# ilovin/lstm_ctc_ocr

Hardware: NVIDIA H100
Metric: text-line images/sec (fwd+CTC loss) (higher is better)
Workload: dtype bf16

## Files before the change

### lstm_ctc_ocr_b200/csrc/backward.cu

```cuda
#include <cmath>
#include <cstring>

#include "backward_kernels.cuh"
#include "conv1_wgrad_tc.cuh"
#include "conv_swap.cuh"
#include "gemm_launch.h"
#include "kernels.cuh"
#include "lstm_bwd.cuh"
#include "model_internal.h"

extern "C" int crnn_model_set_training(crnn_model* m, int flag) {
  if (!m) return crnn_fail(CRNN_INVALID_VALUE, "set_training: null model");
  if (flag && m->cfg.compute_dtype >= 2) return crnn_fail(CRNN_UNSUPPORTED, "set_training: the f32-class paths (compute_dtype 2, 3) are forward + CTC only");
  if (flag && !m->wblock_bwd) {
    const size_t nB[9] = {512 * 4608, 256 * 4608, 256 * 2304, 128 * 2304, 64 * 1152, 1024 * 1024, 512 * 64, 512 * 2048, 512 * 1024};
    size_t tot = 1024;
    for (size_t v : nB) tot += align_up(v * 2);
    CUDA_TRY(cudaMalloc(&m->wblock_bwd, tot));
    uint8_t* p = reinterpret_cast<uint8_t*>(m->wblock_bwd);
    __nv_bfloat16** dst[9] = {&m->Bd_c42, &m->Bd_c41, &m->Bd_c32, &m->Bd_c31, &m->Bd_c2, &m->Bd_c5, &m->Bld, &m->Bxb, &m->Bhb};
    for (int i = 0; i < 9; ++i) { *dst[i] = reinterpret_cast<__nv_bfloat16*>(p); p += align_up(nB[i] * 2); }
    m->grad_sumsq = reinterpret_cast<double*>(p);
    CRNN_TRY(make_tmap_2d(&m->tD_c42, m->Bd_c42, 512, 4608, 4608, 256));
    CRNN_TRY(make_tmap_2d(&m->tD_c41, m->Bd_c41, 256, 4608, 4608, 256));
    CRNN_TRY(make_tmap_2d(&m->tD_c32, m->Bd_c32, 256, 2304, 2304, 256));
    CRNN_TRY(make_tmap_2d(&m->tD_c31, m->Bd_c31, 128, 2304, 2304, 128));
    CRNN_TRY(make_tmap_2d(&m->tD_c2, m->Bd_c2, 64, 1152, 1152, 64));
    CRNN_TRY(make_tmap_2d(&m->tDs_c2, m->Bd_c2, 64, 1152, 1152, 128));
    CRNN_TRY(make_tmap_2d(&m->tD_c5, m->Bd_c5, 1024, 1024, 1024, 256));
    CRNN_TRY(make_tmap_2d(&m->tD_l, m->Bld, 512, 64, 64, 256));
    CRNN_TRY(make_tmap_2d(&m->tD_x, m->Bxb, 512, 2048, 2048, 256));
    CRNN_TRY(make_tmap_2d(&m->tD_h, m->Bhb, 512, 1024, 1024, 32));
    CRNN_TRY(make_tmap_2d(&m->tD_h256, m->Bhb, 512, 1024, 1024, 256));
    m->dirty_bwd = true;
  }
  m->training = flag != 0;
  return CRNN_OK;
}

static int prepare_weights_bwd(crnn_model* m, cudaStream_t st) {
  CRNN_TRY(launch_dgrad_weight(m->P("conv4_2/weights"), m->Bd_c42, 512, 512, st));
  CRNN_TRY(launch_dgrad_weight(m->P("conv4_1/weights"), m->Bd_c41, 256, 512, st));
  CRNN_TRY(launch_dgrad_weight(m->P("conv3_2/weights"), m->Bd_c32, 256, 256, st));
  CRNN_TRY(launch_dgrad_weight(m->P("conv3_1/weights"), m->Bd_c31, 128, 256, st));
  CRNN_TRY(launch_dgrad_weight(m->P("conv2/weights"), m->Bd_c2, 64, 128, st));
  CRNN_TRY(launch_conv5_dgrad_weight(m->P("conv5/weights"), m->Bd_c5, st));
  CRNN_TRY(launch_cast_bf16(m->P("logits/weights"), m->Bld, 512 * 64, st));
  CRNN_TRY(launch_lstm_bwd_weight(m->P("logits/bidirectional_rnn/fw/lstm_cell/weights"), m->P("logits/bidirectional_rnn/bw/lstm_cell/weights"),
                                  m->Bxb, m->Bhb, 32, st));
  m->dirty_bwd = false;
  return CRNN_OK;
}

static gemm_tn::Params tn_plain(int M, int Ncols, long long rows, float* out, long long ldo) {
  gemm_tn::Params p;
  memset(&p, 0, sizeof(p));
  p.num_taps = 1;
  p.num_m_tiles = (M + 127) / 128;
// ... 349 lines not shown
```

### lstm_ctc_ocr_b200/csrc/forward_x3.cu

```cuda
#include <cstring>
#include <string>

#include "gemm_launch.h"
#include "kernels.cuh"
#include "model_internal.h"

namespace x3 {

__device__ __forceinline__ void split2(float v, __nv_bfloat16& hi, __nv_bfloat16& lo) {
  hi = __float2bfloat16_rn(v);
  lo = __float2bfloat16_rn(v - __bfloat162float(hi));
}

__device__ __forceinline__ uint2 pack4(const __nv_bfloat16* h) {
  uint2 r;
  r.x = (uint32_t)__bfloat16_as_ushort(h[0]) | ((uint32_t)__bfloat16_as_ushort(h[1]) << 16);
  r.y = (uint32_t)__bfloat16_as_ushort(h[2]) | ((uint32_t)__bfloat16_as_ushort(h[3]) << 16);
  return r;
}

__global__ void __launch_bounds__(256) split_weight_kernel(const float* __restrict__ src, int K, int Cout, int ld, int inner,
                                                           __nv_bfloat16* __restrict__ dst) {
  const size_t i = (size_t)blockIdx.x * blockDim.x + threadIdx.x;
  if (i >= (size_t)K * Cout) return;
// ... 236 lines not shown
    CRNN_TRY(make_tmap_2d_f32(&pl.tA_l, pl.slo, Rt, 512, 512, 128));
    CRNN_TRY(make_tmap_2d_f32(&pl.tA_h, pl.hS, (uint64_t)2 * pl.Npad, 256, 256, 128));
    return CRNN_OK;
  }
  CRNN_TRY(make_tmap_nhwc(&pl.tA_c2, pl.s1, N, pl.H1, 16, 128, pl.mg2 ? 8 : 2));
  CRNN_TRY(make_tmap_nhwc(&pl.tA_c31, pl.s2, N, pl.H2, 8, 256, pl.mg3 ? 16 : 4));
  CRNN_TRY(make_tmap_nhwc(&pl.tA_c32, pl.s3, N, pl.H2, 8, 512, pl.mg3 ? 16 : 4));
  CRNN_TRY(make_tmap_nhwc(&pl.tA_c41, pl.s3p, N, pl.H2, 4, 512, pl.mg4 ? 32 : 8));
  CRNN_TRY(make_tmap_nhwc(&pl.tA_c42, pl.s4a, N, pl.H2, 4, 1024, pl.mg4 ? 32 : 8));
  const uint64_t R = (uint64_t)N * pl.H2;
  CRNN_TRY(make_tmap_2d(&pl.tA_c5, pl.s4b, R, 2048, 2048, 128));
  CRNN_TRY(make_tmap_2d(&pl.tA_x, pl.s5, R, 1024, 1024, 128));
  CRNN_TRY(make_tmap_2d(&pl.tA_l, pl.slo, R, 1024, 1024, 128));
  CRNN_TRY(make_tmap_2d(&pl.tA_h, pl.hS, (uint64_t)2 * pl.Npad, 512, 512, 128));
  return CRNN_OK;
}

static int prepare(crnn_model* m, State* s, cudaStream_t st) {
  const int kK[9] = {576, 1152, 2304, 2304, 4608, 2048, 512, 256, 512};
  const int kCo[9] = {128, 256, 256, 512, 512, 512, 2048, 2048, 64};
  if (!s->wblock) {
    const size_t eb = s->tf32 ? 4 : 6;
    size_t tot = 0;
    for (int i = 0; i < 9; ++i) tot += align_up((size_t)kK[i] * kCo[i] * eb);
    CUDA_TRY(cudaMalloc(&s->wblock, tot));
    uint8_t* p = reinterpret_cast<uint8_t*>(s->wblock);
    uint8_t** dst[9] = {&s->Bc2, &s->Bc31, &s->Bc32, &s->Bc41, &s->Bc42, &s->Bc5, &s->Bx, &s->Bh, &s->Bl};
    for (int i = 0; i < 9; ++i) { *dst[i] = p; p += align_up((size_t)kK[i] * kCo[i] * eb); }
  }
  if (s->tf32) {
    if (!s->maps_ready) {
      CUtensorMap* tm[9] = {&s->tB_c2, &s->tB_c31, &s->tB_c32, &s->tB_c41, &s->tB_c42, &s->tB_c5, &s->tB_x, &s->tB_h, &s->tB_l};
      uint8_t* base[9] = {s->Bc2, s->Bc31, s->Bc32, s->Bc41, s->Bc42, s->Bc5, s->Bx, s->Bh, s->Bl};
      const int box[9] = {128, 256, 256, 256, 256, 256, 256, 256, 64};
      for (int i = 0; i < 9; ++i) CRNN_TRY(make_tmap_2d_f32(tm[i], base[i], kCo[i], kK[i], kK[i], box[i]));
      s->maps_ready = true;
    }
    auto tw = [&](const float* src, int K, int Cout, int ld, uint8_t* dst) -> int {
      const size_t n = (size_t)K * Cout;
      tf32_weight_kernel<<<(unsigned)((n + 255) / 256), 256, 0, st>>>(src, K, Cout, ld, reinterpret_cast<float*>(dst));
      CUDA_TRY(cudaGetLastError());
      return CRNN_OK;
    };
    CRNN_TRY(tw(m->P("conv2/weights"), 576, 128, 128, s->Bc2));
    CRNN_TRY(tw(m->P("conv3_1/weights"), 1152, 256, 256, s->Bc31));
    CRNN_TRY(tw(m->P("conv3_2/weights"), 2304, 256, 256, s->Bc32));
    CRNN_TRY(tw(m->P("conv4_1/weights"), 2304, 512, 512, s->Bc41));
    CRNN_TRY(tw(m->P("conv4_2/weights"), 4608, 512, 512, s->Bc42));
    CRNN_TRY(tw(m->P("conv5/weights"), 2048, 512, 512, s->Bc5));
    const char* dn[2] = {"logits/bidirectional_rnn/fw/lstm_cell/weights", "logits/bidirectional_rnn/bw/lstm_cell/weights"};
    for (int d = 0; d < 2; ++d) {
      const float* w = m->P(dn[d]);
      CRNN_TRY(tw(w, 512, 1024, 1024, s->Bx + (size_t)d * 1024 * 512 * 4));
      CRNN_TRY(tw(w + 512 * 1024, 256, 1024, 1024, s->Bh + (size_t)d * 1024 * 256 * 4));
    }
    CRNN_TRY(tw(m->P("logits/weights"), 512, 64, 64, s->Bl));
    s->dirty = false;
    return CRNN_OK;
  }
  if (!s->maps_ready) {
    s->maps_ready = true;
    CRNN_TRY(make_tmap_2d(&s->tB_c2, s->Bc2, 128, 1728, 1728, 128));
    CRNN_TRY(make_tmap_2d(&s->tB_c31, s->Bc31, 256, 3456, 3456, 256));
    CRNN_TRY(make_tmap_2d(&s->tB_c32, s->Bc32, 256, 6912, 6912, 256));
    CRNN_TRY(make_tmap_2d(&s->tB_c41, s->Bc41, 512, 6912, 6912, 256));
    CRNN_TRY(make_tmap_2d(&s->tB_c42, s->Bc42, 512, 13824, 13824, 256));
    CRNN_TRY(make_tmap_2d(&s->tB_c5, s->Bc5, 512, 6144, 6144, 256));
    CRNN_TRY(make_tmap_2d(&s->tB_x, s->Bx, 2048, 1536, 1536, 256));
    CRNN_TRY(make_tmap_2d(&s->tB_h, s->Bh, 2048, 768, 768, 256));
    CRNN_TRY(make_tmap_2d(&s->tB_l, s->Bl, 64, 1536, 1536, 64));
  }
  auto sw = [&](const float* src, int K, int Cout, int ld, int inner, uint8_t* dst) -> int {
    const size_t n = (size_t)K * Cout;
    split_weight_kernel<<<(unsigned)((n + 255) / 256), 256, 0, st>>>(src, K, Cout, ld, inner, reinterpret_cast<__nv_bfloat16*>(dst));
    CUDA_TRY(cudaGetLastError());
    return CRNN_OK;
  };
  CRNN_TRY(sw(m->P("conv2/weights"), 576, 128, 128, 64, s->Bc2));
  CRNN_TRY(sw(m->P("conv3_1/weights"), 1152, 256, 256, 128, s->Bc31));
  CRNN_TRY(sw(m->P("conv3_2/weights"), 2304, 256, 256, 256, s->Bc32));
  CRNN_TRY(sw(m->P("conv4_1/weights"), 2304, 512, 512, 256, s->Bc41));
  CRNN_TRY(sw(m->P("conv4_2/weights"), 4608, 512, 512, 512, s->Bc42));
  CRNN_TRY(sw(m->P("conv5/weights"), 2048, 512, 512, 1024, s->Bc5));
  const char* dirs[2] = {"logits/bidirectional_rnn/fw/lstm_cell/weights", "logits/bidirectional_rnn/bw/lstm_cell/weights"};
  for (int d = 0; d < 2; ++d) {
    const float* w = m->P(dirs[d]);
    CRNN_TRY(sw(w, 512, 1024, 1024, 512, s->Bx + (size_t)d * 1024 * 1536 * 2));
    CRNN_TRY(sw(w + 512 * 1024, 256, 1024, 1024, 256, s->Bh + (size_t)d * 1024 * 768 * 2));
  }
  CRNN_TRY(sw(m->P("logits/weights"), 512, 64, 64, 512, s->Bl));
  s->dirty = false;
  return CRNN_OK;
}

template <int POOL>
static int act_split(bool tf, const float* in, void* out, const float* bias, const float* scale, const float* shift, int relu, int Nimg,
                     int H, int Wd, int C, int G, cudaStream_t st) {
  const int Ho = (POOL == 1) ? H / 2 : H, Wo = (POOL != 0) ? Wd / 2 : Wd;
  const size_t total = (size_t)Nimg * Ho * Wo * (C / 4);
// ... 187 lines not shown
```

### lstm_ctc_ocr_b200/csrc/gemm.cuh

```cuda
#pragma once
#include <cuda.h>

#include "common.cuh"
#include "wgmma.cuh"

namespace gemm {

constexpr int BLOCK_M = 128;
constexpr int BLOCK_K = 64;
constexpr int UMMA_K = 16;
constexpr int A_STAGE_BYTES = BLOCK_M * 128;
constexpr int NUM_THREADS = 384;
constexpr int MAX_SMEM = 232448;

enum AMode { A_PLAIN = 0, A_CONV3 = 1 };
enum Epi {
  EPI_F32 = 0,
  EPI_BIAS_BF16 = 1,
  EPI_RELU = 2,
  EPI_RELU_POOL22 = 3,
  EPI_RELU_POOL12 = 4,
  EPI_STATS = 5,
  EPI_LSTM = 6,
  EPI_LOGITS = 7,
// ... 55 lines not shown
  for (int i = 0; i < 4; ++i) {
    float send = (lane & 4) ? r8[i] : r8[i + 4];
    float keep = (lane & 4) ? r8[i + 4] : r8[i];
    r4[i] = keep + __shfl_xor_sync(0xffffffffu, send, 4);
  }
#pragma unroll
  for (int i = 0; i < 2; ++i) {
    float send = (lane & 2) ? r4[i] : r4[i + 2];
    float keep = (lane & 2) ? r4[i + 2] : r4[i];
    r2[i] = keep + __shfl_xor_sync(0xffffffffu, send, 2);
  }
  float send = (lane & 1) ? r2[0] : r2[1];
  float keep = (lane & 1) ? r2[1] : r2[0];
  return keep + __shfl_xor_sync(0xffffffffu, send, 1);
}

constexpr int slice_cols(int block_n, int epi) {
  return (block_n < 256 || epi == EPI_LSTM || epi == EPI_CONV_STORE_BNRED) ? block_n
       : (epi == EPI_RELU || epi == EPI_STATS || epi == EPI_BIAS_BF16 || epi == EPI_XPROJ || epi == EPI_CONV_STORE) ? 128 : 64;
}

template <int BLOCK_N, int STAGES, int SLICE_N>
struct Smem {
  static constexpr int B_STAGE_BYTES = BLOCK_N * 128;
  static constexpr int ACC_BYTES = BLOCK_M * SLICE_N * 4;
  static constexpr int FIT = (MAX_SMEM - ACC_BYTES - 256 - 1024) / (A_STAGE_BYTES + B_STAGE_BYTES);
  static constexpr int S = STAGES < FIT ? STAGES : FIT;
  static constexpr int ACC_OFFSET = S * (A_STAGE_BYTES + B_STAGE_BYTES);
  static constexpr int BAR_OFFSET = ACC_OFFSET + ACC_BYTES;
  static constexpr int BYTES = BAR_OFFSET + 256 + 1024;
};
static_assert(Smem<256, 4, 64>::S == 4, "a 64-column staging slice leaves room for a 4-stage ring at BLOCK_N = 256");

constexpr bool frag_epi(int block_n, int epi) {
  return block_n == 256 && (epi == EPI_RELU || epi == EPI_RELU_POOL12 || epi == EPI_STATS || epi == EPI_BIAS_BF16 ||
                            epi == EPI_XPROJ || epi == EPI_CONV_STORE);
}

__device__ __forceinline__ uint32_t* stg_word(uint8_t* buf, int box_bytes, int row, int c) {
  return reinterpret_cast<uint32_t*>(buf + (c >> 6) * box_bytes + row * 128 + ((((c >> 3) & 7) ^ (row & 7)) << 4) + ((c & 7) << 1));
}

template <int W>
__device__ __forceinline__ float4 rowsum_tree(const uint8_t* box, int rg, int cw, int i) {
  if constexpr (W == 32) {
    const int r = rg * 32 + i;
    const uint32_t v = *reinterpret_cast<const uint32_t*>(box + r * 128 + (((cw >> 2) ^ (r & 7)) << 4) + ((cw & 3) << 2));
    const float x = ptx::bf16_lo(v), y = ptx::bf16_hi(v);
    return make_float4(x, y, __fmul_rn(x, x), __fmul_rn(y, y));
  } else {
    const float4 a = rowsum_tree<W * 2>(box, rg, cw, i), b = rowsum_tree<W * 2>(box, rg, cw, i + W);
    return make_float4(a.x + b.x, a.y + b.y, a.z + b.z, a.w + b.w);
  }
}

template <bool LINES>
__device__ __forceinline__ bool conv_row_valid(const Params& p, int m_blk, int r) {
  const int g = m_blk * 4 + (r >> 5);
  const int n_img = g / p.sb_per_img;
  const int h = (g - n_img * p.sb_per_img) * p.bh + (r & 31) / p.Wd;
  if (LINES) return n_img < p.Nimg && h < (__ldg(p.line_w + n_img) >> 2);
  return n_img < p.Nimg && h < p.H;
}

template <int EPI, bool LINES = false>
__device__ __forceinline__ void frag_epilogue(const Params& p, const float (&d)[128], uint8_t* stg, const CUtensorMap* tmO,
// ... 456 lines not shown
        const uint32_t* xfw = reinterpret_cast<const uint32_t*>(xf);
        const uint32_t* xow = reinterpret_cast<const uint32_t*>(xo);
        float* cpf = reinterpret_cast<float*>(cp);
        float hv[16];
#pragma unroll
        for (int i = 0; i < 16; ++i) {
          const float zi = __uint_as_float(gi[i]) + ((i & 1) ? ptx::bf16_hi(xiw[i >> 1]) : ptx::bf16_lo(xiw[i >> 1]));
          const float zj = __uint_as_float(gj[i]) + ((i & 1) ? ptx::bf16_hi(xjw[i >> 1]) : ptx::bf16_lo(xjw[i >> 1]));
          const float zf = __uint_as_float(gf[i]) + ((i & 1) ? ptx::bf16_hi(xfw[i >> 1]) : ptx::bf16_lo(xfw[i >> 1]));
          const float zo = __uint_as_float(go[i]) + ((i & 1) ? ptx::bf16_hi(xow[i >> 1]) : ptx::bf16_lo(xow[i >> 1]));
          const float c = ptx::fast_sigmoid(zf) * cpf[i] + ptx::fast_sigmoid(zi) * ptx::fast_tanh(zj);
          cpf[i] = c;
          hv[i] = ptx::fast_sigmoid(zo) * ptx::fast_tanh(c);
        }
#pragma unroll
        for (int i = 0; i < 4; ++i) *(reinterpret_cast<float4*>(cst + u0) + i) = cp[i];
#pragma unroll
        for (int i = 0; i < 8; ++i) hp[i] = ptx::pack_bf16x2(hv[2 * i], hv[2 * i + 1]);
      } else {
#pragma unroll
        for (int i = 0; i < 8; ++i) hp[i] = 0u;
      }
      if (okn) {
        *reinterpret_cast<uint4*>(hn + u0) = make_uint4(hp[0], hp[1], hp[2], hp[3]);
        *reinterpret_cast<uint4*>(hn + u0 + 8) = make_uint4(hp[4], hp[5], hp[6], hp[7]);
        *reinterpret_cast<uint4*>(lo + u0) = make_uint4(hp[0], hp[1], hp[2], hp[3]);
        *reinterpret_cast<uint4*>(lo + u0 + 8) = make_uint4(hp[4], hp[5], hp[6], hp[7]);
      }
    }
  }

}

template <int BLOCK_N, int AMODE, int EPI, int STAGES, int KIND = 0, bool LINES = false>
__global__ void __launch_bounds__(NUM_THREADS, 1)
gemm_kernel(const __grid_constant__ CUtensorMap tmA, const __grid_constant__ CUtensorMap tmB, const __grid_constant__ CUtensorMap tmO,
            const Params p) {
  static_assert(BLOCK_N == 64 || BLOCK_N == 128 || BLOCK_N == 256, "BLOCK_N");
  constexpr bool FRAG = frag_epi(BLOCK_N, EPI);
  static_assert(!LINES || (FRAG && AMODE == A_CONV3 && KIND == 0), "line masks exist in the register-side conv epilogues only");
  constexpr int SLICE_N = slice_cols(BLOCK_N, EPI);
  using SM = Smem<BLOCK_N, STAGES, SLICE_N>;
  constexpr int S = SM::S;
  constexpr int B_STAGE_BYTES = BLOCK_N * 128;
  constexpr int KELEMS = KIND ? 32 : BLOCK_K;

  extern __shared__ uint8_t smem_raw[];
  uint8_t* smem = reinterpret_cast<uint8_t*>((reinterpret_cast<uintptr_t>(smem_raw) + 1023) & ~uintptr_t(1023));
  uint8_t* smem_a = smem;
  uint8_t* smem_b = smem + S * A_STAGE_BYTES;
  float* acc_tile = reinterpret_cast<float*>(smem + SM::ACC_OFFSET);
  uint64_t* full_bar = reinterpret_cast<uint64_t*>(smem + SM::BAR_OFFSET);
  uint64_t* empty_bar = full_bar + S;

  const int warp_idx = threadIdx.x >> 5;
  const int lane = threadIdx.x & 31;
  const int num_tiles = p.num_m_tiles * p.num_n_tiles;

  if (warp_idx == 0 && lane == 0) {
    ptx::prefetch_tmap(&tmA);
    ptx::prefetch_tmap(&tmB);
    if (FRAG) ptx::prefetch_tmap(&tmO);
    for (int s = 0; s < S; ++s) {
      ptx::mbar_init(&full_bar[s], 1);
      ptx::mbar_init(&empty_bar[s], 2);
    }
    ptx::fence_barrier_init();
  }
  __syncthreads();

  if (warp_idx < 4) {
    ptx::setmaxnreg_dec<24>();
    const int nA = (AMODE == A_CONV3 && !p.merged) ? 4 : 1;
    if (warp_idx == 0 && lane <= nA) {
      int stage = 0;
      uint32_t phase = 0;
      for (int tile = blockIdx.x; tile < num_tiles; tile += gridDim.x) {
        const int m_blk = p.m_tile0 + tile / p.num_n_tiles, n_blk = tile % p.num_n_tiles;
        int b_row = n_blk * BLOCK_N;
        if (EPI == EPI_LSTM) b_row += (m_blk >= p.m_tiles_per_dir) ? 1024 : 0;
        int cn = 0, ch0 = 0;
        if (AMODE == A_CONV3 && lane < nA) {
          const int g = m_blk * 4 + lane;
          cn = g / p.sb_per_img;
          ch0 = (g - cn * p.sb_per_img) * p.bh;
        }
        int tap = 0, cb = 0;
        for (int kb = 0; kb < p.num_k_blocks; ++kb) {
          ptx::mbar_wait(&empty_bar[stage], phase ^ 1);
          if (p.debug_skip_tma) {
            if (lane == 0) ptx::mbar_arrive(&full_bar[stage]);
          } else {
            if (lane == 0) ptx::mbar_arrive_expect_tx(&full_bar[stage], A_STAGE_BYTES + B_STAGE_BYTES);
            if (lane < nA) {
              uint8_t* a_dst = smem_a + stage * A_STAGE_BYTES;
              if (AMODE == A_PLAIN) {
                const int rs = kb / p.kb_per_shift;
                int kc = kb - rs * p.kb_per_shift;
                if (p.kb_phys > 0 && kc >= p.kb_phys) kc -= p.kb_phys;
                ptx::tma_load_2d(&tmA, &full_bar[stage], a_dst, kc * KELEMS, m_blk * BLOCK_M + rs * p.row_shift_mul);
              } else {
                const int r = tap / 3, sx = tap - 3 * r;
                const int cbp = (p.cin_phys > 0 && cb >= p.cin_phys) ? cb - p.cin_phys : cb;
                ptx::tma_load_4d(&tmA, &full_bar[stage], a_dst + lane * 4096, cbp * KELEMS, sx - 1, ch0 + r - 1, cn);
              }
            } else {
              ptx::tma_load_2d(&tmB, &full_bar[stage], smem_b + stage * B_STAGE_BYTES, kb * KELEMS, b_row);
            }
          }
          if (++cb == p.cin_blocks) { cb = 0; ++tap; }
          if (++stage == S) { stage = 0; phase ^= 1; }
        }
      }
    }
  } else {
    ptx::setmaxnreg_inc<240>();
    const int wgi = (warp_idx >> 2) - 1;
    const int q = warp_idx & 3;
    const int chalf = (warp_idx - 4) >> 2;
    const bool arriver = (warp_idx & 3) == 0 && lane == 0;
    const bool issuer = FRAG && threadIdx.x == 128;
    int stage = 0;
    uint32_t phase = 0;
    for (int tile = blockIdx.x; tile < num_tiles; tile += gridDim.x) {
      const int m_blk = p.m_tile0 + tile / p.num_n_tiles, n_blk = tile % p.num_n_tiles;
      float d[BLOCK_N / 2];
      int prev = -1;
      for (int kb = 0; kb < p.num_k_blocks; ++kb) {
        ptx::mbar_wait(&full_bar[stage], phase);
        const uint64_t a_desc = ptx::make_desc_k_sw128(ptx::smem_u32(smem_a + stage * A_STAGE_BYTES + wgi * 64 * 128));
        const uint64_t b_desc = ptx::make_desc_k_sw128(ptx::smem_u32(smem_b + stage * B_STAGE_BYTES));
        wg::fence();
#pragma unroll
        for (int k = 0; k < BLOCK_K / UMMA_K; ++k) {
          if (KIND) wg::mma_tf32<BLOCK_N>(d, a_desc + 2 * k, b_desc + 2 * k, (kb | k) != 0);
          else wg::mma_bf16<BLOCK_N>(d, a_desc + 2 * k, b_desc + 2 * k, (kb | k) != 0);
        }
        wg::commit();
        wg::wait<1>();
        if (prev >= 0 && arriver) ptx::mbar_arrive(&empty_bar[prev]);
        prev = stage;
        if (++stage == S) { stage = 0; phase ^= 1; }
      }
      wg::wait<0>();
      wg::fence_operand(d);
      if (prev >= 0 && arriver) ptx::mbar_arrive(&empty_bar[prev]);
      if (p.debug_skip_epilogue) continue;
      if constexpr (FRAG) {
        frag_epilogue<EPI, LINES>(p, d, reinterpret_cast<uint8_t*>(acc_tile), &tmO, m_blk, n_blk, wgi, issuer);
      } else {
#pragma unroll
        for (int s = 0; s < BLOCK_N / SLICE_N; ++s) {
          ptx::bar_sync(1, 256);
          ptx::acc_store_slice<BLOCK_N, SLICE_N>(acc_tile, d, wgi * 64, s);
          ptx::bar_sync(1, 256);
          const int c_lo = s * SLICE_N + chalf * (SLICE_N / 2);
          run_epilogue<BLOCK_N, SLICE_N, EPI>(p, acc_tile, m_blk, n_blk, q, lane, c_lo, c_lo + SLICE_N / 2, s * SLICE_N);
        }
      }
    }
    if (FRAG && issuer) ptx::bulk_wait_all();
  }
}

}
```

### lstm_ctc_ocr_b200/csrc/gemm_launch.h

```cpp
#pragma once
#include "gemm.cuh"
#include "gemm_tn.cuh"
#include <cstdlib>
#include <string>

template <int BN, int AM, int EPI, int ST, int KIND = 0, bool LINES = false>
static int launch_gemm(const CUtensorMap& a, const CUtensorMap& b, const gemm::Params& p, int num_sms, cudaStream_t st,
                       const CUtensorMap* out = nullptr) {
  if (gemm::frag_epi(BN, EPI) && out == nullptr) return crnn_fail(CRNN_INVALID_VALUE, "launch_gemm: epilogue %d needs an output tensor map", EPI);
  auto kern = gemm::gemm_kernel<BN, AM, EPI, ST, KIND, LINES>;
  constexpr int smem = gemm::Smem<BN, ST, gemm::slice_cols(BN, EPI)>::BYTES;
  static bool attr = false;
  if (!attr) {
    CUDA_TRY(cudaFuncSetAttribute(kern, cudaFuncAttributeMaxDynamicSharedMemorySize, smem));
    attr = true;
  }
  const int tiles = p.num_m_tiles * p.num_n_tiles;
  const int grid = tiles < num_sms ? tiles : num_sms;
  kern<<<grid, gemm::NUM_THREADS, smem, st>>>(a, b, out ? *out : a, p);
  CUDA_TRY(cudaGetLastError());
  return CRNN_OK;
}

static inline int pick_k_splits(int tiles, int k_blocks_total, int workers) {
  static const bool old_rule = [] { const char* e = getenv("CRNN_KSPLIT"); return e && std::string(e) == "old"; }();
  if (old_rule) {
    int s = (3 * workers + tiles - 1) / tiles;
    if (s > k_blocks_total) s = k_blocks_total;
    return s < 1 ? 1 : s;
  }
  const int kEpi = 6;
  int best = 1;
  long long best_cost = -1;
  const int kmax = k_blocks_total < 4 * workers ? k_blocks_total : 4 * workers;
  for (int k = 1; k <= kmax; ++k) {
    const long long rounds = ((long long)tiles * k + workers - 1) / workers;
    const long long cost = rounds * ((k_blocks_total + k - 1) / k + kEpi);
    if (best_cost < 0 || cost < best_cost) { best_cost = cost; best = k; }
  }
  return best;
}

template <int BN, int AM, int ST>
static int launch_gemm_tn(const CUtensorMap& a, const CUtensorMap& b, gemm_tn::Params p, int num_sms, cudaStream_t st) {
  auto kern = gemm_tn::gemm_tn_kernel<BN, AM, ST>;
  constexpr int smem = gemm_tn::Smem<BN, ST>::BYTES;
  static bool attr = false;
  if (!attr) {
    CUDA_TRY(cudaFuncSetAttribute(kern, cudaFuncAttributeMaxDynamicSharedMemorySize, smem));
    attr = true;
  }
  const int tiles = p.num_taps * p.num_m_tiles * p.num_n_tiles;
// ... 8 lines not shown
```

### lstm_ctc_ocr_b200/csrc/model.cu

```cuda
#include <cstdarg>
#include <cstring>
#include <string>
#include <vector>

#include <cstdlib>
#include <condition_variable>
#include <mutex>
#include <thread>

#include "gemm_launch.h"
#include "lstm.cuh"
#include "conv_swap.cuh"
#include "conv1_tc.cuh"
#include "kernels.cuh"
#include "model_internal.h"

static thread_local char g_err[1024] = "";
int crnn_fail(int status, const char* fmt, ...) {
  va_list ap;
  va_start(ap, fmt);
  vsnprintf(g_err, sizeof(g_err), fmt, ap);
  va_end(ap);
  return status;
}
// ... 144 lines not shown
    delete m;
    return crnn_fail(CRNN_CUDA_ERROR, "model_create: no CUDA device (this library has no CPU fallback)");
  }
  if (prop.major != 9) {
    delete m;
    return crnn_fail(CRNN_UNSUPPORTED, "model_create: needs sm_90 (found sm_%d%d)", prop.major, prop.minor);
  }
  m->num_sms = prop.multiProcessorCount;
  if (const char* e = getenv("CRNN_BPTT")) m->bptt_ks = std::string(e) != "ring";
  if (const char* e = getenv("CRNN_CONV1")) m->conv1_tc = std::string(e) != "simt";
  if (const char* e = getenv("CRNN_BN_FUSE")) m->bn_red_fused = std::string(e) != "0";
  if (const char* e = getenv("CRNN_RELU_FUSE")) m->relu_mask_fused = std::string(e) != "0";
  if (const char* e = getenv("CRNN_CONV1_WGRAD")) m->conv1_wgrad_tc = std::string(e) != "simt";
  if (const char* e = getenv("CRNN_CONV2_DGRAD")) m->conv2_dgrad_swap = std::string(e) != "old";
  if (const char* e = getenv("CRNN_CONV2_WGRAD")) m->conv2_wgrad_swap = std::string(e) != "old";
  if (const char* e = getenv("CRNN_CONV2")) m->conv2_swap = std::string(e) != "pos";
  if (const char* e = getenv("CRNN_LSTM_IMPL")) {
    m->lstm_upc = (std::string(e) == "step") ? 64 : 32;
    m->lstm_mc = std::string(e) == "ds" ? 2 : std::string(e) == "mc" ? 1 : std::string(e) == "gx" ? 4 : (std::string(e) == "persistent" || std::string(e) == "step") ? 0 : 3;
  }

  const size_t nB[9] = {128 * 576, 256 * 1152, 256 * 2304, 512 * 2304, 512 * 4608, 512 * 2048, 2048 * 512, 2048 * 256, 64 * 512};
  size_t tot = 0;
  for (size_t v : nB) tot += (v * 2 + 1023) / 1024 * 1024;
  tot += 2048 * 4 + 1024;
  if (cudaMalloc(&m->wblock, tot) != cudaSuccess) { delete m; return crnn_fail(CRNN_CUDA_ERROR, "model_create: cudaMalloc"); }
  uint8_t* p = reinterpret_cast<uint8_t*>(m->wblock);
  __nv_bfloat16** dst[9] = {&m->Bc2, &m->Bc31, &m->Bc32, &m->Bc41, &m->Bc42, &m->Bc5, &m->Bx, &m->Bh, &m->Bl};
  for (int i = 0; i < 9; ++i) { *dst[i] = reinterpret_cast<__nv_bfloat16*>(p); p += (nB[i] * 2 + 1023) / 1024 * 1024; }
  m->xbias = reinterpret_cast<float*>(p); p += 2048 * 4;
  m->sumsq = reinterpret_cast<double*>(p);
  int st = CRNN_OK;
  if (st == CRNN_OK) st = make_tmap_2d(&m->tB_c2, m->Bc2, 128, 576, 576, 128);
  if (st == CRNN_OK) st = make_tmap_2d(&m->tB_c31, m->Bc31, 256, 1152, 1152, 256);
  if (st == CRNN_OK) st = make_tmap_2d(&m->tB_c32, m->Bc32, 256, 2304, 2304, 256);
  if (st == CRNN_OK) st = make_tmap_2d(&m->tB_c41, m->Bc41, 512, 2304, 2304, 256);
  if (st == CRNN_OK) st = make_tmap_2d(&m->tB_c42, m->Bc42, 512, 4608, 4608, 256);
  if (st == CRNN_OK) st = make_tmap_2d(&m->tB_c5, m->Bc5, 512, 2048, 2048, 256);
  if (st == CRNN_OK) st = make_tmap_2d(&m->tB_x, m->Bx, 2048, 512, 512, 256);
  if (st == CRNN_OK) st = make_tmap_2d(&m->tB_h, m->Bh, 2048, 256, 256, 256);
  if (st == CRNN_OK) st = make_tmap_2d(&m->tB_h128, m->Bh, 2048, 256, 256, 128);
  if (st == CRNN_OK) st = make_tmap_2d(&m->tB_l, m->Bl, 64, 512, 512, 64);
  if (st != CRNN_OK) { cudaFree(m->wblock); delete m; return st; }
  *out = m;
  return CRNN_OK;
}

extern "C" int crnn_model_destroy(crnn_model* m) {
  if (!m) return CRNN_OK;
  x3_destroy(m);
  if (m->wblock) cudaFree(m->wblock);
  if (m->wblock_bwd) cudaFree(m->wblock_bwd);
  if (m->d_peers) cudaFree(m->d_peers);
  for (auto e : m->prof_events) cudaEventDestroy(e);
  for (auto e : m->prof_events_bwd) cudaEventDestroy(e);
  for (auto e : m->chunk_events) cudaEventDestroy(e);
  delete m;
  return CRNN_OK;
}
extern "C" int crnn_num_tensors(const crnn_model* m) { return m ? (int)m->tensors.size() : 0; }
extern "C" int64_t crnn_param_count(const crnn_model* m) { return m ? m->total : 0; }
extern "C" int crnn_param_info(const crnn_model* m, int index, const char** tf_name, int64_t* offset, int64_t shape[4],
                               int* ndim) {
  if (!m || index < 0 || index >= (int)m->tensors.size()) return crnn_fail(CRNN_INVALID_VALUE, "param_info: bad index");
  const TensorInfo& t = m->tensors[index];
  if (tf_name) *tf_name = t.name.c_str();
  if (offset) *offset = t.offset;
  if (shape) for (int k = 0; k < 4; ++k) shape[k] = t.shape[k];
  if (ndim) *ndim = t.ndim;
  return CRNN_OK;
// ... 658 lines not shown
  if (!m || !name || !dst) return crnn_fail(CRNN_INVALID_VALUE, "debug_tap_raw: null");
  if (m->cfg.compute_dtype >= 2) return x3_debug_tap_raw(m, name, dst, dst_bytes, workspace, reinterpret_cast<cudaStream_t>(stream));
  Plan& pl = m->plan;
  if (pl.ws == nullptr || pl.ws != workspace) return crnn_fail(CRNN_INVALID_VALUE, "debug_tap_raw: no forward ran on this workspace");
  const size_t n = pl.N, h1 = pl.H1, h2 = pl.H2;
  const void* src = nullptr;
  size_t bytes = 0;
  bool train_only = false;
  std::string s(name);
  if (s == "bn" && pl.line_w) { src = pl.bn_l; bytes = 2 * n * 4 * 512 * sizeof(float); }
  else if (s == "stats" && pl.line_w) { src = pl.stats_l; bytes = 2 * n * 2 * 512 * sizeof(double); }
  else if (s == "bn") { src = pl.bn; bytes = 2 * 4 * 512 * sizeof(float); }
  else if (s == "stats") { src = pl.stats; bytes = 2 * 2 * 512 * sizeof(double); }
  else if (s == "am1") { src = pl.am1; bytes = n * h1 * 16 * 64; train_only = true; }
  else if (s == "am2") { src = pl.am2; bytes = n * h2 * 8 * 128; train_only = true; }
  else if (s == "am3") { src = pl.am3; bytes = n * h2 * 4 * 256; train_only = true; }
  else if (s == "csave") { src = pl.csave; bytes = (size_t)2 * pl.Npad * pl.T * 256 * sizeof(float); train_only = true; }
  else return crnn_fail(CRNN_INVALID_VALUE, "debug_tap_raw: unknown tap %s", name);
  if (train_only && !pl.train) return crnn_fail(CRNN_INVALID_VALUE, "debug_tap_raw: %s exists only in a training-mode plan", name);
  if (dst_bytes < bytes) return crnn_fail(CRNN_INVALID_VALUE, "debug_tap_raw: dst too small (%zu < %zu bytes)", dst_bytes, bytes);
  CUDA_TRY(cudaMemcpyAsync(dst, src, bytes, cudaMemcpyDeviceToDevice, reinterpret_cast<cudaStream_t>(stream)));
  return CRNN_OK;
}

extern "C" int crnn_test_gemm_bf16(const void* A, const void* B, float* D, int M, int Nc, int K, int block_n,
                                   crnn_stream_t stream) {
  if (!A || !B || !D || M <= 0 || Nc <= 0 || K <= 0 || (K % 64) != 0 || (Nc % block_n) != 0)
    return crnn_fail(CRNN_INVALID_VALUE, "test_gemm: bad args");
  int dev = 0, sms = 132;
  cudaGetDevice(&dev);
  cudaDeviceGetAttribute(&sms, cudaDevAttrMultiProcessorCount, dev);
  CUtensorMap ta, tb;
  CRNN_TRY(make_tmap_2d(&ta, A, M, K, K, 128));
  CRNN_TRY(make_tmap_2d(&tb, B, Nc, K, K, block_n));
  gemm::Params p;
  memset(&p, 0, sizeof(p));
  p.M = M; p.Nc = Nc;
  p.num_m_tiles = (M + 127) / 128; p.num_n_tiles = Nc / block_n; p.num_k_blocks = K / 64; p.kb_per_shift = p.num_k_blocks;
  p.out = D;
  if (const char* e = getenv("CRNN_PROBE_SKIP_TMA")) p.debug_skip_tma = (e[0] == '1');
  if (const char* e = getenv("CRNN_PROBE_SKIP_EPI")) p.debug_skip_epilogue = (e[0] == '1');
  cudaStream_t st = reinterpret_cast<cudaStream_t>(stream);
  if (const char* e = getenv("CRNN_PROBE_BF16_OUT"); e && e[0] == '1' && block_n == 256) {
    CUtensorMap to;
    CRNN_TRY(make_tmap_2d(&to, D, M, Nc, Nc, 128));
    p.ldo = Nc;
    return launch_gemm<256, gemm::A_PLAIN, gemm::EPI_BIAS_BF16, 4>(ta, tb, p, sms, st, &to);
  }
  if (block_n == 64) return launch_gemm<64, gemm::A_PLAIN, gemm::EPI_F32, 8>(ta, tb, p, sms, st);
  if (block_n == 128) return launch_gemm<128, gemm::A_PLAIN, gemm::EPI_F32, 6>(ta, tb, p, sms, st);
  if (block_n == 256) return launch_gemm<256, gemm::A_PLAIN, gemm::EPI_F32, 4>(ta, tb, p, sms, st);
  return crnn_fail(CRNN_INVALID_VALUE, "test_gemm: block_n must be 64/128/256");
}
```

### lstm_ctc_ocr_b200/csrc/ptx.cuh

```cuda
#pragma once
#include <cuda_runtime.h>
#include <cuda_bf16.h>
#include <stdint.h>

namespace ptx {

__device__ __forceinline__ uint32_t smem_u32(const void* p) {
  return static_cast<uint32_t>(__cvta_generic_to_shared(p));
}
__device__ __forceinline__ uint32_t lane_id() { return threadIdx.x & 31; }

__device__ __forceinline__ bool elect_one() {
  uint32_t pred = 0;
  asm volatile(
      "{\n\t.reg .pred p;\n\t"
      "elect.sync _|p, 0xffffffff;\n\t"
      "selp.u32 %0, 1, 0, p;\n\t}\n"
      : "=r"(pred));
  return pred != 0;
}

__device__ __forceinline__ void mbar_init(uint64_t* bar, uint32_t count) {
  asm volatile("mbarrier.init.shared::cta.b64 [%0], %1;" ::"r"(smem_u32(bar)), "r"(count));
}
// ... 145 lines not shown
  }
}


__device__ __forceinline__ uint32_t cluster_ctarank() {
  uint32_t r;
  asm volatile("mov.u32 %0, %%cluster_ctarank;" : "=r"(r));
  return r;
}
__device__ __forceinline__ void cluster_sync_all() {
  asm volatile("barrier.cluster.arrive.release.aligned;" ::: "memory");
  asm volatile("barrier.cluster.wait.acquire.aligned;" ::: "memory");
}
__device__ __forceinline__ uint32_t mapa(uint32_t local_smem_addr, uint32_t rank) {
  uint32_t r;
  asm volatile("mapa.shared::cluster.u32 %0, %1, %2;" : "=r"(r) : "r"(local_smem_addr), "r"(rank));
  return r;
}
__device__ __forceinline__ void mbar_wait_cluster(uint64_t* bar, uint32_t parity) {
  uint32_t ok;
  do {
    asm volatile(
        "{\n\t.reg .pred p;\n\t"
        "mbarrier.try_wait.parity.acquire.cluster.shared::cta.b64 p, [%1], %2;\n\t"
        "selp.u32 %0, 1, 0, p;\n\t}\n"
        : "=r"(ok)
        : "r"(smem_u32(bar)), "r"(parity)
        : "memory");
  } while (!ok);
}
__device__ __forceinline__ void mbar_arrive_cluster(uint32_t cluster_addr) {
  asm volatile("mbarrier.arrive.release.cluster.shared::cluster.b64 _, [%0];" ::"r"(cluster_addr) : "memory");
}
__device__ __forceinline__ void tma_load_2d_mc(const void* tmap, uint64_t* bar, void* dst, int c0, int c1, uint16_t cta_mask) {
  asm volatile(
      "cp.async.bulk.tensor.2d.shared::cluster.global.tile.mbarrier::complete_tx::bytes.multicast::cluster [%0], [%1, {%3, %4}], [%2], %5;"
      ::"r"(smem_u32(dst)), "l"(reinterpret_cast<uint64_t>(tmap)), "r"(smem_u32(bar)), "r"(c0), "r"(c1), "h"(cta_mask)
      : "memory");
}
__device__ __forceinline__ uint32_t pack_bf16x2(float lo, float hi) {
  __nv_bfloat162 t = __floats2bfloat162_rn(lo, hi);
  return *reinterpret_cast<uint32_t*>(&t);
}
__device__ __forceinline__ uint32_t hmax2_bf16(uint32_t a, uint32_t b) {
  __nv_bfloat162 x = *reinterpret_cast<__nv_bfloat162*>(&a);
  __nv_bfloat162 y = *reinterpret_cast<__nv_bfloat162*>(&b);
  __nv_bfloat162 r = __hmax2(x, y);
  return *reinterpret_cast<uint32_t*>(&r);
}
__device__ __forceinline__ float bf16_lo(uint32_t v) { return __uint_as_float(v << 16); }
__device__ __forceinline__ float bf16_hi(uint32_t v) { return __uint_as_float(v & 0xFFFF0000u); }

__device__ __forceinline__ void st_global_v8(void* ptr, uint32_t a, uint32_t b, uint32_t c, uint32_t d, uint32_t e, uint32_t f,
                                             uint32_t g, uint32_t h) {
  uint4* p = reinterpret_cast<uint4*>(ptr);
  p[0] = make_uint4(a, b, c, d);
  p[1] = make_uint4(e, f, g, h);
}

__device__ __forceinline__ uint64_t pack_f32x2(float lo, float hi) {
  uint64_t r;
  asm("mov.b64 %0, {%1, %2};" : "=l"(r) : "f"(lo), "f"(hi));
  return r;
}
__device__ __forceinline__ void unpack_f32x2(uint64_t v, float& lo, float& hi) {
  asm("mov.b64 {%0, %1}, %2;" : "=f"(lo), "=f"(hi) : "l"(v));
// ... 26 lines not shown
```

Baseline: 180,100.

## Multicast conv weight tiles across 2-CTA clusters in BLOCK_N=256 conv GEMMs

Conv3-mode GEMMs with BLOCK_N=256 now launch as 2-CTA clusters. The CTAs in a cluster work on adjacent M tiles and split the B (weight) stage load, each issuing a TMA multicast of half the rows to both CTAs. Weight tensor-map boxes for conv3_1 through conv4_2 shrink to 128 rows to match. Empty-barrier release becomes a remote arrive on every CTA in the cluster. The aim is to halve L2 to shared-memory weight traffic, at the cost of cluster scheduling limits, cross-CTA barrier coupling, and idle padded tiles when the M-tile count is odd.

```diff
diff --git a/lstm_ctc_ocr_b200/csrc/backward.cu b/lstm_ctc_ocr_b200/csrc/backward.cu
--- a/lstm_ctc_ocr_b200/csrc/backward.cu
+++ b/lstm_ctc_ocr_b200/csrc/backward.cu
@@ -21,9 +21,9 @@
     __nv_bfloat16** dst[9] = {&m->Bd_c42, &m->Bd_c41, &m->Bd_c32, &m->Bd_c31, &m->Bd_c2, &m->Bd_c5, &m->Bld, &m->Bxb, &m->Bhb};
     for (int i = 0; i < 9; ++i) { *dst[i] = reinterpret_cast<__nv_bfloat16*>(p); p += align_up(nB[i] * 2); }
     m->grad_sumsq = reinterpret_cast<double*>(p);
-    CRNN_TRY(make_tmap_2d(&m->tD_c42, m->Bd_c42, 512, 4608, 4608, 256));
-    CRNN_TRY(make_tmap_2d(&m->tD_c41, m->Bd_c41, 256, 4608, 4608, 256));
-    CRNN_TRY(make_tmap_2d(&m->tD_c32, m->Bd_c32, 256, 2304, 2304, 256));
+    CRNN_TRY(make_tmap_2d(&m->tD_c42, m->Bd_c42, 512, 4608, 4608, 128));
+    CRNN_TRY(make_tmap_2d(&m->tD_c41, m->Bd_c41, 256, 4608, 4608, 128));
+    CRNN_TRY(make_tmap_2d(&m->tD_c32, m->Bd_c32, 256, 2304, 2304, 128));
     CRNN_TRY(make_tmap_2d(&m->tD_c31, m->Bd_c31, 128, 2304, 2304, 128));
     CRNN_TRY(make_tmap_2d(&m->tD_c2, m->Bd_c2, 64, 1152, 1152, 64));
     CRNN_TRY(make_tmap_2d(&m->tDs_c2, m->Bd_c2, 64, 1152, 1152, 128));
diff --git a/lstm_ctc_ocr_b200/csrc/forward_x3.cu b/lstm_ctc_ocr_b200/csrc/forward_x3.cu
--- a/lstm_ctc_ocr_b200/csrc/forward_x3.cu
+++ b/lstm_ctc_ocr_b200/csrc/forward_x3.cu
@@ -292,7 +292,7 @@
     if (!s->maps_ready) {
       CUtensorMap* tm[9] = {&s->tB_c2, &s->tB_c31, &s->tB_c32, &s->tB_c41, &s->tB_c42, &s->tB_c5, &s->tB_x, &s->tB_h, &s->tB_l};
       uint8_t* base[9] = {s->Bc2, s->Bc31, s->Bc32, s->Bc41, s->Bc42, s->Bc5, s->Bx, s->Bh, s->Bl};
-      const int box[9] = {128, 256, 256, 256, 256, 256, 256, 256, 64};
+      const int box[9] = {128, 128, 128, 128, 128, 256, 256, 256, 64};
       for (int i = 0; i < 9; ++i) CRNN_TRY(make_tmap_2d_f32(tm[i], base[i], kCo[i], kK[i], kK[i], box[i]));
       s->maps_ready = true;
     }
@@ -321,10 +321,10 @@
   if (!s->maps_ready) {
     s->maps_ready = true;
     CRNN_TRY(make_tmap_2d(&s->tB_c2, s->Bc2, 128, 1728, 1728, 128));
-    CRNN_TRY(make_tmap_2d(&s->tB_c31, s->Bc31, 256, 3456, 3456, 256));
-    CRNN_TRY(make_tmap_2d(&s->tB_c32, s->Bc32, 256, 6912, 6912, 256));
-    CRNN_TRY(make_tmap_2d(&s->tB_c41, s->Bc41, 512, 6912, 6912, 256));
-    CRNN_TRY(make_tmap_2d(&s->tB_c42, s->Bc42, 512, 13824, 13824, 256));
+    CRNN_TRY(make_tmap_2d(&s->tB_c31, s->Bc31, 256, 3456, 3456, 128));
+    CRNN_TRY(make_tmap_2d(&s->tB_c32, s->Bc32, 256, 6912, 6912, 128));
+    CRNN_TRY(make_tmap_2d(&s->tB_c41, s->Bc41, 512, 6912, 6912, 128));
+    CRNN_TRY(make_tmap_2d(&s->tB_c42, s->Bc42, 512, 13824, 13824, 128));
     CRNN_TRY(make_tmap_2d(&s->tB_c5, s->Bc5, 512, 6144, 6144, 256));
     CRNN_TRY(make_tmap_2d(&s->tB_x, s->Bx, 2048, 1536, 1536, 256));
     CRNN_TRY(make_tmap_2d(&s->tB_h, s->Bh, 2048, 768, 768, 256));
diff --git a/lstm_ctc_ocr_b200/csrc/gemm.cuh b/lstm_ctc_ocr_b200/csrc/gemm.cuh
--- a/lstm_ctc_ocr_b200/csrc/gemm.cuh
+++ b/lstm_ctc_ocr_b200/csrc/gemm.cuh
@@ -111,6 +111,8 @@
 };
 static_assert(Smem<256, 4, 64>::S == 4, "a 64-column staging slice leaves room for a 4-stage ring at BLOCK_N = 256");
 
+constexpr int cluster_ctas(int block_n, int amode) { return (block_n == 256 && amode == A_CONV3) ? 2 : 1; }
+
 constexpr bool frag_epi(int block_n, int epi) {
   return block_n == 256 && (epi == EPI_RELU || epi == EPI_RELU_POOL12 || epi == EPI_STATS || epi == EPI_BIAS_BF16 ||
                             epi == EPI_XPROJ || epi == EPI_CONV_STORE);
@@ -633,7 +635,7 @@
 
 }
 
-template <int BLOCK_N, int AMODE, int EPI, int STAGES, int KIND = 0, bool LINES = false>
+template <int BLOCK_N, int AMODE, int EPI, int STAGES, int KIND = 0, bool LINES = false, int CTAS = cluster_ctas(BLOCK_N, AMODE)>
 __global__ void __launch_bounds__(NUM_THREADS, 1)
 gemm_kernel(const __grid_constant__ CUtensorMap tmA, const __grid_constant__ CUtensorMap tmB, const __grid_constant__ CUtensorMap tmO,
             const Params p) {
@@ -645,6 +647,7 @@
   constexpr int S = SM::S;
   constexpr int B_STAGE_BYTES = BLOCK_N * 128;
   constexpr int KELEMS = KIND ? 32 : BLOCK_K;
+  static_assert(CTAS == 1 || ((CTAS == 2 || CTAS == 4) && BLOCK_N == 256 && EPI != EPI_LSTM), "clusters: N = 256, B rows independent of the M tile");
 
   extern __shared__ uint8_t smem_raw[];
   uint8_t* smem = reinterpret_cast<uint8_t*>((reinterpret_cast<uintptr_t>(smem_raw) + 1023) & ~uintptr_t(1023));
@@ -656,7 +659,14 @@
 
   const int warp_idx = threadIdx.x >> 5;
   const int lane = threadIdx.x & 31;
-  const int num_tiles = p.num_m_tiles * p.num_n_tiles;
+  const int rank = blockIdx.x % CTAS;
+  const int num_units = (p.num_m_tiles + CTAS - 1) / CTAS * p.num_n_tiles;
+  auto tile_of = [&](int u, int& m_blk, int& n_blk) {
+    const int m_local = (u / p.num_n_tiles) * CTAS + rank;
+    m_blk = p.m_tile0 + m_local;
+    n_blk = u % p.num_n_tiles;
+    return m_local < p.num_m_tiles;
+  };
 
   if (warp_idx == 0 && lane == 0) {
     ptx::prefetch_tmap(&tmA);
@@ -664,11 +674,12 @@
     if (FRAG) ptx::prefetch_tmap(&tmO);
     for (int s = 0; s < S; ++s) {
       ptx::mbar_init(&full_bar[s], 1);
-      ptx::mbar_init(&empty_bar[s], 2);
+      ptx::mbar_init(&empty_bar[s], 2 * CTAS);
     }
     ptx::fence_barrier_init();
   }
-  __syncthreads();
+  if (CTAS > 1) ptx::cluster_sync_all();
+  else __syncthreads();
 
   if (warp_idx < 4) {
     ptx::setmaxnreg_dec<24>();
@@ -676,8 +687,9 @@
     if (warp_idx == 0 && lane <= nA) {
       int stage = 0;
       uint32_t phase = 0;
-      for (int tile = blockIdx.x; tile < num_tiles; tile += gridDim.x) {
-        const int m_blk = p.m_tile0 + tile / p.num_n_tiles, n_blk = tile % p.num_n_tiles;
+      for (int u = blockIdx.x / CTAS; u < num_units; u += gridDim.x / CTAS) {
+        int m_blk, n_blk;
+        tile_of(u, m_blk, n_blk);
         int b_row = n_blk * BLOCK_N;
         if (EPI == EPI_LSTM) b_row += (m_blk >= p.m_tiles_per_dir) ? 1024 : 0;
         int cn = 0, ch0 = 0;
@@ -705,6 +717,10 @@
                 const int cbp = (p.cin_phys > 0 && cb >= p.cin_phys) ? cb - p.cin_phys : cb;
                 ptx::tma_load_4d(&tmA, &full_bar[stage], a_dst + lane * 4096, cbp * KELEMS, sx - 1, ch0 + r - 1, cn);
               }
+            } else if (CTAS > 1) {
+              constexpr int HALF = B_STAGE_BYTES / CTAS;
+              ptx::tma_load_2d_mc(&tmB, &full_bar[stage], smem_b + stage * B_STAGE_BYTES + rank * HALF, kb * KELEMS,
+                                  b_row + rank * (BLOCK_N / CTAS), (1 << CTAS) - 1);
             } else {
               ptx::tma_load_2d(&tmB, &full_bar[stage], smem_b + stage * B_STAGE_BYTES, kb * KELEMS, b_row);
             }
@@ -721,10 +737,19 @@
     const int chalf = (warp_idx - 4) >> 2;
     const bool arriver = (warp_idx & 3) == 0 && lane == 0;
     const bool issuer = FRAG && threadIdx.x == 128;
+    auto release = [&](int s) {
+      if (CTAS == 1) {
+        ptx::mbar_arrive(&empty_bar[s]);
+      } else {
+#pragma unroll
+        for (int c = 0; c < CTAS; ++c) ptx::mbar_arrive_remote(ptx::mapa(ptx::smem_u32(&empty_bar[s]), c));
+      }
+    };
     int stage = 0;
     uint32_t phase = 0;
-    for (int tile = blockIdx.x; tile < num_tiles; tile += gridDim.x) {
-      const int m_blk = p.m_tile0 + tile / p.num_n_tiles, n_blk = tile % p.num_n_tiles;
+    for (int u = blockIdx.x / CTAS; u < num_units; u += gridDim.x / CTAS) {
+      int m_blk, n_blk;
+      const bool real = tile_of(u, m_blk, n_blk);
       float d[BLOCK_N / 2];
       int prev = -1;
       for (int kb = 0; kb < p.num_k_blocks; ++kb) {
@@ -739,14 +764,14 @@
         }
         wg::commit();
         wg::wait<1>();
-        if (prev >= 0 && arriver) ptx::mbar_arrive(&empty_bar[prev]);
+        if (prev >= 0 && arriver) release(prev);
         prev = stage;
         if (++stage == S) { stage = 0; phase ^= 1; }
       }
       wg::wait<0>();
       wg::fence_operand(d);
-      if (prev >= 0 && arriver) ptx::mbar_arrive(&empty_bar[prev]);
-      if (p.debug_skip_epilogue) continue;
+      if (prev >= 0 && arriver) release(prev);
+      if (p.debug_skip_epilogue || !real) continue;
       if constexpr (FRAG) {
         frag_epilogue<EPI, LINES>(p, d, reinterpret_cast<uint8_t*>(acc_tile), &tmO, m_blk, n_blk, wgi, issuer);
       } else {
@@ -762,6 +787,10 @@
     }
     if (FRAG && issuer) ptx::bulk_wait_all();
   }
-}
-
-}
+  if (CTAS > 1) {
+    __syncwarp();
+    ptx::cluster_sync_all();
+  }
+}
+
+}
diff --git a/lstm_ctc_ocr_b200/csrc/gemm_launch.h b/lstm_ctc_ocr_b200/csrc/gemm_launch.h
--- a/lstm_ctc_ocr_b200/csrc/gemm_launch.h
+++ b/lstm_ctc_ocr_b200/csrc/gemm_launch.h
@@ -2,22 +2,47 @@
 #include "gemm.cuh"
 #include "gemm_tn.cuh"
 #include <cstdlib>
+#include <cstring>
 #include <string>
 
-template <int BN, int AM, int EPI, int ST, int KIND = 0, bool LINES = false>
+template <int BN, int AM, int EPI, int ST, int KIND = 0, bool LINES = false, int CTAS = gemm::cluster_ctas(BN, AM)>
 static int launch_gemm(const CUtensorMap& a, const CUtensorMap& b, const gemm::Params& p, int num_sms, cudaStream_t st,
                        const CUtensorMap* out = nullptr) {
   if (gemm::frag_epi(BN, EPI) && out == nullptr) return crnn_fail(CRNN_INVALID_VALUE, "launch_gemm: epilogue %d needs an output tensor map", EPI);
-  auto kern = gemm::gemm_kernel<BN, AM, EPI, ST, KIND, LINES>;
+  auto kern = gemm::gemm_kernel<BN, AM, EPI, ST, KIND, LINES, CTAS>;
   constexpr int smem = gemm::Smem<BN, ST, gemm::slice_cols(BN, EPI)>::BYTES;
+  constexpr int ctas = CTAS;
+  cudaLaunchConfig_t cfg;
+  memset(&cfg, 0, sizeof(cfg));
+  cfg.blockDim = dim3(gemm::NUM_THREADS);
+  cfg.dynamicSmemBytes = smem;
+  cfg.stream = st;
+  cudaLaunchAttribute at[1];
+  at[0].id = cudaLaunchAttributeClusterDimension;
+  at[0].val.clusterDim.x = ctas; at[0].val.clusterDim.y = 1; at[0].val.clusterDim.z = 1;
+  cfg.attrs = at; cfg.numAttrs = 1;
   static bool attr = false;
+  static int max_clusters = 0;
   if (!attr) {
     CUDA_TRY(cudaFuncSetAttribute(kern, cudaFuncAttributeMaxDynamicSharedMemorySize, smem));
+    if (ctas > 1) {
+      cfg.gridDim = dim3(ctas);
+      CUDA_TRY(cudaOccupancyMaxActiveClusters(&max_clusters, kern, &cfg));
+      if (max_clusters < 1) return crnn_fail(CRNN_CUDA_ERROR, "launch_gemm: no %d-CTA cluster of epilogue %d fits on the device", ctas, EPI);
+    }
     attr = true;
   }
-  const int tiles = p.num_m_tiles * p.num_n_tiles;
-  const int grid = tiles < num_sms ? tiles : num_sms;
-  kern<<<grid, gemm::NUM_THREADS, smem, st>>>(a, b, out ? *out : a, p);
+  const int units = (p.num_m_tiles + ctas - 1) / ctas * p.num_n_tiles;
+  int workers = num_sms / ctas;
+  if (ctas > 1 && workers > max_clusters) workers = max_clusters;
+  if (workers < 1) workers = 1;
+  const int grid = ctas * (units < workers ? units : workers);
+  if (ctas == 1) {
+    kern<<<grid, gemm::NUM_THREADS, smem, st>>>(a, b, out ? *out : a, p);
+  } else {
+    cfg.gridDim = dim3(grid);
+    CUDA_TRY(cudaLaunchKernelEx(&cfg, kern, a, b, out ? *out : a, p));
+  }
   CUDA_TRY(cudaGetLastError());
   return CRNN_OK;
 }
diff --git a/lstm_ctc_ocr_b200/csrc/model.cu b/lstm_ctc_ocr_b200/csrc/model.cu
--- a/lstm_ctc_ocr_b200/csrc/model.cu
+++ b/lstm_ctc_ocr_b200/csrc/model.cu
@@ -200,10 +200,10 @@
   m->sumsq = reinterpret_cast<double*>(p);
   int st = CRNN_OK;
   if (st == CRNN_OK) st = make_tmap_2d(&m->tB_c2, m->Bc2, 128, 576, 576, 128);
-  if (st == CRNN_OK) st = make_tmap_2d(&m->tB_c31, m->Bc31, 256, 1152, 1152, 256);
-  if (st == CRNN_OK) st = make_tmap_2d(&m->tB_c32, m->Bc32, 256, 2304, 2304, 256);
-  if (st == CRNN_OK) st = make_tmap_2d(&m->tB_c41, m->Bc41, 512, 2304, 2304, 256);
-  if (st == CRNN_OK) st = make_tmap_2d(&m->tB_c42, m->Bc42, 512, 4608, 4608, 256);
+  if (st == CRNN_OK) st = make_tmap_2d(&m->tB_c31, m->Bc31, 256, 1152, 1152, 128);
+  if (st == CRNN_OK) st = make_tmap_2d(&m->tB_c32, m->Bc32, 256, 2304, 2304, 128);
+  if (st == CRNN_OK) st = make_tmap_2d(&m->tB_c41, m->Bc41, 512, 2304, 2304, 128);
+  if (st == CRNN_OK) st = make_tmap_2d(&m->tB_c42, m->Bc42, 512, 4608, 4608, 128);
   if (st == CRNN_OK) st = make_tmap_2d(&m->tB_c5, m->Bc5, 512, 2048, 2048, 256);
   if (st == CRNN_OK) st = make_tmap_2d(&m->tB_x, m->Bx, 2048, 512, 512, 256);
   if (st == CRNN_OK) st = make_tmap_2d(&m->tB_h, m->Bh, 2048, 256, 256, 256);
@@ -928,7 +928,7 @@
   cudaDeviceGetAttribute(&sms, cudaDevAttrMultiProcessorCount, dev);
   CUtensorMap ta, tb;
   CRNN_TRY(make_tmap_2d(&ta, A, M, K, K, 128));
-  CRNN_TRY(make_tmap_2d(&tb, B, Nc, K, K, block_n));
+  CRNN_TRY(make_tmap_2d(&tb, B, Nc, K, K, block_n == 256 ? 128 : block_n));
   gemm::Params p;
   memset(&p, 0, sizeof(p));
   p.M = M; p.Nc = Nc;
@@ -941,10 +941,10 @@
     CUtensorMap to;
     CRNN_TRY(make_tmap_2d(&to, D, M, Nc, Nc, 128));
     p.ldo = Nc;
-    return launch_gemm<256, gemm::A_PLAIN, gemm::EPI_BIAS_BF16, 4>(ta, tb, p, sms, st, &to);
+    return launch_gemm<256, gemm::A_PLAIN, gemm::EPI_BIAS_BF16, 4, 0, false, 2>(ta, tb, p, sms, st, &to);
   }
   if (block_n == 64) return launch_gemm<64, gemm::A_PLAIN, gemm::EPI_F32, 8>(ta, tb, p, sms, st);
   if (block_n == 128) return launch_gemm<128, gemm::A_PLAIN, gemm::EPI_F32, 6>(ta, tb, p, sms, st);
-  if (block_n == 256) return launch_gemm<256, gemm::A_PLAIN, gemm::EPI_F32, 4>(ta, tb, p, sms, st);
+  if (block_n == 256) return launch_gemm<256, gemm::A_PLAIN, gemm::EPI_F32, 4, 0, false, 2>(ta, tb, p, sms, st);
   return crnn_fail(CRNN_INVALID_VALUE, "test_gemm: block_n must be 64/128/256");
 }
diff --git a/lstm_ctc_ocr_b200/csrc/ptx.cuh b/lstm_ctc_ocr_b200/csrc/ptx.cuh
--- a/lstm_ctc_ocr_b200/csrc/ptx.cuh
+++ b/lstm_ctc_ocr_b200/csrc/ptx.cuh
@@ -201,6 +201,9 @@
 __device__ __forceinline__ void mbar_arrive_cluster(uint32_t cluster_addr) {
   asm volatile("mbarrier.arrive.release.cluster.shared::cluster.b64 _, [%0];" ::"r"(cluster_addr) : "memory");
 }
+__device__ __forceinline__ void mbar_arrive_remote(uint32_t cluster_addr) {
+  asm volatile("mbarrier.arrive.shared::cluster.b64 _, [%0];" ::"r"(cluster_addr) : "memory");
+}
 __device__ __forceinline__ void tma_load_2d_mc(const void* tmap, uint64_t* bar, void* dst, int c0, int c1, uint16_t cta_mask) {
   asm volatile(
       "cp.async.bulk.tensor.2d.shared::cluster.global.tile.mbarrier::complete_tx::bytes.multicast::cluster [%0], [%1, {%3, %4}], [%2], %5;"
```

Measured after the change: 180,800 (median of 6 runs). No clear change (+0.4%).
